# francescoalemanno/KissABC.jl

Hardware: AMD Instinct MI355X
Metric: walker proposal+cost evals/sec at N=65536 walkers, D=8 (higher is better)
Workload: dtype f64

## Files before the change

### include/kabc.h

```cpp
#ifndef KABC_H
#define KABC_H

#ifndef __HIPCC_RTC__
#include <stddef.h>
#include <stdint.h>
#else
#include "kabc_rtc_types.h"
#endif

#ifdef __cplusplus
extern "C" {
#endif

#define KABC_VERSION 321
#define KABC_MAX_DIM 16
#define KABC_MAX_DIM_DYN 256

typedef enum kabc_status {
    KABC_OK = 0,
    KABC_ERR_INVALID_ARG = 1,
    KABC_ERR_RETRY_EXHAUSTED = 2,
    KABC_ERR_INVALID_STATE = 3,
    KABC_ERR_DEVICE = 4,
    KABC_ERR_UNSUPPORTED = 5,
// ... 97 lines not shown
    int64_t keep;
    uint64_t seed;
    int64_t first_row;
} kabc_reject_opts_t;

typedef struct kabc_reject_result {
    double* theta;
    double* cost;
    double* logprior;
    int64_t* index;
    int64_t capacity;
    int64_t n_out;
    int64_t draws;
    int64_t accepted_seen;
    double eps;
    int32_t exhausted;
    int32_t course;
    int64_t launches;
    double kernel_ms;
} kabc_reject_result_t;

void kabc_reject_default_opts(kabc_reject_opts_t* opts);
kabc_status_t kabc_abc_reject(kabc_ctx_t* ctx, const kabc_prior_t* prior, int32_t D, const kabc_cost_t* cost,
                              const kabc_reject_opts_t* opts, kabc_reject_result_t* result);

kabc_status_t kabc_abc_reject_batch(kabc_ctx_t* ctx, const kabc_prior_t* prior, int32_t D,
                                    const kabc_cost_t* costs, int64_t nruns, const uint64_t* seeds,
                                    const double* eps, const kabc_reject_opts_t* opts,
                                    kabc_reject_result_t* results, kabc_status_t* status);
void kabc_reject_batch_stats(int64_t out[4]);

kabc_status_t kabc_math_probe(kabc_ctx_t* ctx, int32_t fn, int64_t n, const double* x,
                              double* out);

kabc_status_t kabc_poison_probe(kabc_ctx_t* ctx, int64_t n, uint8_t* fresh, uint8_t* pooled,
                                uint8_t* recycled, int32_t info[2]);

kabc_status_t kabc_register_cost_plugin(const char* path, int32_t* out_cost_id);
kabc_status_t kabc_compile_cost_plugin(const char* src, const int32_t* dims, int32_t ndims,
                                       int32_t posterior_mask, int32_t* out_cost_id);
kabc_status_t kabc_plugin_precompile(int32_t cost_id, int32_t family, int32_t D, int32_t variant);

kabc_status_t kabc_compile_prior_plugin(const char* src, int32_t discrete, int32_t* out_kind);

kabc_status_t kabc_compile_mvprior_plugin(const char* src, int32_t* out_kind);

#define KABC_FAMILY_AIS 1
#define KABC_FAMILY_SMC 2
#define KABC_FAMILY_ABCDE 4
#define KABC_FAMILY_PFILTER 8
#define KABC_FAMILY_AIS_SMALL 16
kabc_status_t kabc_compile_model(const kabc_model_t* model, int32_t families, int32_t* out_handle);
kabc_status_t kabc_model_release(int32_t handle);
kabc_status_t kabc_prefetch_model(const kabc_model_t* model, int32_t families);
#define KABC_SPECIALIZE_ENV (-1)
#define KABC_SPECIALIZE_OFF 0
#define KABC_SPECIALIZE_BLOCKING 1
#define KABC_SPECIALIZE_BACKGROUND 2
kabc_status_t kabc_set_specialize(int32_t mode);
int32_t kabc_rtc_cache_dir(char* out, int32_t cap);
#define KABC_SPEC_NONE 0
#define KABC_SPEC_PENDING 1
#define KABC_SPEC_ACTIVE 2
#define KABC_SPEC_FAILED 3
kabc_status_t kabc_spec_counters(uint64_t out[4]);
int32_t kabc_rtc_worker_main(const char* jobfile);
// ... 280 lines not shown
```

### kissabc.jl_amd/_cdefs.py

```python
import ctypes as C

KABC_MAX_DIM = 16
KABC_MAX_DIM_DYN = 256
KABC_VERSION = 321
KABC_COMM_ID_BYTES = 128
KABC_MAX_EXCHANGE_CHUNKS = 16
KABC_COMM_MAX_WORLD = 16
COMM_RCCL, COMM_P2P = 1, 2

KABC_OK, KABC_ERR_INVALID_ARG, KABC_ERR_RETRY_EXHAUSTED, KABC_ERR_INVALID_STATE, \
    KABC_ERR_DEVICE, KABC_ERR_UNSUPPORTED, KABC_ERR_NAN_COST, KABC_ERR_CANCELLED = range(8)

PRIOR_UNIFORM, PRIOR_NORMAL, PRIOR_TRUNCNORMAL, PRIOR_BETA, PRIOR_DISCRETE_UNIFORM, \
    PRIOR_NEGBINOMIAL, PRIOR_EXPONENTIAL, PRIOR_GAMMA, PRIOR_LOGNORMAL = range(1, 10)
PRIOR_USER_INIT = 10
PRIOR_MVNORMAL = 11
PRIOR_USER = 100
FAMILY_AIS, FAMILY_SMC, FAMILY_ABCDE, FAMILY_PFILTER, FAMILY_AIS_SMALL = 1, 2, 4, 8, 16

POSTERIOR_KERNELIZED, POSTERIOR_THRESHOLD, POSTERIOR_COMMON = 1, 2, 3
SUMMARY_AUTO, SUMMARY_FULL, SUMMARY_DIAG = 0, 1, 2

COST_GAUSS_DIST, COST_ROSENBROCK, COST_HIER_GAUSS_SIM, COST_NORMAL_MEANSTD_SIM, COST_DIRAC_SQ, \
    COST_ABS_DIFF, COST_NORM_SHELL, COST_NOISY_QUAD_DU, COST_MIXTURE, COST_NOISY_BANANA, \
# ... 92 lines not shown

class RejectOpts(C.Structure):
    _fields_ = [("eps", C.c_double), ("n_accept", C.c_int64), ("max_draws", C.c_int64), ("keep", C.c_int64),
                ("seed", C.c_uint64), ("first_row", C.c_int64)]


class RejectResult(C.Structure):
    _fields_ = [("theta", c_double_p), ("cost", c_double_p), ("logprior", c_double_p),
                ("index", C.POINTER(C.c_int64)), ("capacity", C.c_int64), ("n_out", C.c_int64),
                ("draws", C.c_int64), ("accepted_seen", C.c_int64), ("eps", C.c_double),
                ("exhausted", C.c_int32), ("course", C.c_int32), ("launches", C.c_int64),
                ("kernel_ms", C.c_double)]


ABI_REJECT_OPTS, ABI_REJECT_RESULT = 32, 33

VP = C.c_void_p
PROTOTYPES = {
    "kabc_version": (C.c_int32, []),
    "kabc_abi_sizeof": (C.c_int32, [C.c_int32]),
    "kabc_abi_offsetof": (C.c_int32, [C.c_int32, C.c_int32]),
    "kabc_mvnormal_register": (C.c_int, [c_double_p, c_double_p, C.c_int32, C.POINTER(C.c_int32)]),
    "kabc_last_error": (C.c_char_p, []),
    "kabc_device_count": (C.c_int32, []),
    "kabc_ctx_create": (C.c_int, [C.c_int32, VP, C.POINTER(VP)]),
    "kabc_ctx_destroy": (C.c_int, [VP]),
    "kabc_ctx_synchronize": (C.c_int, [VP]),
    "kabc_ctx_cancel": (C.c_int, [VP]),
    "kabc_ctx_clear_cancel": (C.c_int, [VP]),
    "kabc_ctx_cancel_on_sigint": (C.c_int, [VP, C.c_int32]),
    "kabc_math_probe": (C.c_int, [VP, C.c_int32, C.c_int64, c_double_p, c_double_p]),
    "kabc_poison_probe": (C.c_int, [VP, C.c_int64, C.POINTER(C.c_uint8), C.POINTER(C.c_uint8),
                                    C.POINTER(C.c_uint8), C.POINTER(C.c_int32)]),
    "kabc_host_alloc": (C.c_int, [C.c_size_t, C.POINTER(VP)]),
    "kabc_host_free": (C.c_int, [VP]),
    "kabc_factored_logpdf": (C.c_int, [VP, C.POINTER(Prior), C.c_int32, C.c_int64, c_double_p,
                                       c_double_p]),
    "kabc_factored_push_p": (C.c_int, [VP, C.POINTER(Prior), C.c_int32, C.c_int64, c_double_p,
                                       c_double_p]),
    "kabc_factored_rand": (C.c_int, [VP, C.POINTER(Prior), C.c_int32, C.c_uint64, C.c_uint32,
                                     C.c_int64, C.c_int64, C.c_uint64, c_double_p]),
    "kabc_cost_eval": (C.c_int, [VP, C.POINTER(Cost), C.c_int32, C.c_int64, c_double_p, C.c_int32,
                                 C.c_uint64, C.c_int64, c_double_p]),
    "kabc_prior_predictive": (C.c_int, [VP, C.POINTER(Prior), C.c_int32, C.POINTER(Cost), C.c_int64,
                                        C.c_int32, C.c_uint64, C.c_int64, c_double_p, c_double_p,
                                        c_double_p]),
    "kabc_eval_stats": (None, [c_double_p]),
    "kabc_reject_default_opts": (None, [C.POINTER(RejectOpts)]),
    "kabc_abc_reject": (C.c_int, [VP, C.POINTER(Prior), C.c_int32, C.POINTER(Cost), C.POINTER(RejectOpts),
                                  C.POINTER(RejectResult)]),
    "kabc_abc_reject_batch": (C.c_int, [VP, C.POINTER(Prior), C.c_int32, C.POINTER(Cost), C.c_int64,
                                        C.POINTER(C.c_uint64), c_double_p, C.POINTER(RejectOpts),
                                        C.POINTER(RejectResult), C.POINTER(C.c_int)]),
    "kabc_reject_batch_stats": (None, [C.POINTER(C.c_int64)]),
    "kabc_register_cost_plugin": (C.c_int, [C.c_char_p, C.POINTER(C.c_int32)]),
    "kabc_plugin_precompile": (C.c_int, [C.c_int32, C.c_int32, C.c_int32, C.c_int32]),
    "kabc_compile_cost_plugin": (C.c_int, [C.c_char_p, C.POINTER(C.c_int32), C.c_int32, C.c_int32,
                                         C.POINTER(C.c_int32)]),
    "kabc_compile_prior_plugin": (C.c_int, [C.c_char_p, C.c_int32, C.POINTER(C.c_int32)]),
    "kabc_compile_mvprior_plugin": (C.c_int, [C.c_char_p, C.POINTER(C.c_int32)]),
    "kabc_compile_model": (C.c_int, [C.POINTER(Model), C.c_int32, C.POINTER(C.c_int32)]),
    "kabc_model_release": (C.c_int, [C.c_int32]),
    "kabc_prefetch_model": (C.c_int, [C.POINTER(Model), C.c_int32]),
    "kabc_spec_counters": (C.c_int, [C.POINTER(C.c_uint64)]),
    "kabc_set_specialize": (C.c_int, [C.c_int32]),
    "kabc_rtc_cache_dir": (C.c_int32, [C.c_char_p, C.c_int32]),
# ... 100 lines not shown
```

### kissabc.jl_amd/csrc/ais_inst.hip

```cpp
#define KABC_FMA_C_VGPR
#include "ais_small_kernel.hpp"

#ifndef KABC_INST_COST
#error "compile with -DKABC_INST_COST=<cost id>"
#endif

namespace kabc {

template <int D, int COST, int PC, int PK>
static void launch_half(const AisArgs& a, hipStream_t s, unsigned nchains) {
    const unsigned grid = (unsigned)((a.rows_owned + kBatch - 1) / kBatch);
    if (grid == 0) return;
    hipLaunchKernelGGL((ais_half_kernel<D, COST, PC, PK>), dim3(grid, nchains), dim3(kAisBlock), 0, s, a);
}

template <int D, int COST, int PC, int PK, int K, int NC>
static void launch_half_wide(const AisArgs& a, hipStream_t s, unsigned nchains) {
    const dim3 grid = ais_wide_geom(a, nchains);
    if (grid.x == 0) return;
    hipLaunchKernelGGL((ais_half_wide_kernel<D, COST, PC, PK, K, NC>), grid, dim3(kWideBlock), 0, s, a);
}

#ifndef KABC_INST_DLO
#define KABC_INST_DLO 1
#endif
#ifndef KABC_INST_DHI
#define KABC_INST_DHI KABC_MAX_DIM
#endif
#ifndef KABC_INST_SUFFIX
#define KABC_INST_SUFFIX
#endif
#ifndef KABC_INST_PCSEL
#define KABC_INST_PCSEL 0
#endif
template <int COST, int D, int PCX>
static AisLaunchFn pick() {
    constexpr bool is_normal = (PCX % kPriorClasses) == kPriorNormal;
    constexpr bool pc_ok = KABC_INST_PCSEL == 0 || (KABC_INST_PCSEL == 1) == is_normal;
    if constexpr (pc_ok && D >= KABC_INST_DLO && D <= KABC_INST_DHI && cost_dim_ok_c(COST, D))
        return &launch_half<D, COST, PCX % kPriorClasses, PCX / kPriorClasses + 1>;
    else return nullptr;
}

template <int COST, int D, int PCX>
static AisLaunchFn pick_wide() {
    constexpr bool is_normal = (PCX % kPriorClasses) == kPriorNormal;
    constexpr bool pc_ok = KABC_INST_PCSEL == 0 || (KABC_INST_PCSEL == 1) == is_normal;
    if constexpr (pc_ok && D >= KABC_INST_DLO && D <= KABC_INST_DHI && cost_dim_ok_c(COST, D) &&
                  ais_wide_ok_c(COST, D))
        return &launch_half_wide<D, COST, PCX % kPriorClasses, PCX / kPriorClasses + 1, kWideK, kWideNC>;
    else return nullptr;
}

template <int COST, int PCX, bool WIDE, int... Ds>
static AisLaunchFn row(int D, std::integer_sequence<int, Ds...>) {
    AisLaunchFn f[] = {(WIDE ? pick_wide<COST, Ds + 1, PCX>() : pick<COST, Ds + 1, PCX>())...};
    return (D >= 1 && D <= (int)sizeof...(Ds)) ? f[D - 1] : nullptr;
}

template <int COST, bool WIDE, int... PCXs>
static AisLaunchFn table(int D, int pcx, std::integer_sequence<int, PCXs...>) {
    using Dims = std::make_integer_sequence<int, KABC_MAX_DIM>;
    AisLaunchFn r = nullptr;
    ((pcx == PCXs ? (void)(r = row<COST, PCXs, WIDE>(D, Dims{})) : (void)0), ...);
    return r;
}

template <int COST, int D, int PCX>
static AisSmallLaunchFn pick_small() {
    constexpr int pc = PCX % kPriorClasses;
    constexpr bool is_normal = pc == kPriorNormal;
    constexpr bool pc_ok = KABC_INST_PCSEL == 0 || (KABC_INST_PCSEL == 1) == is_normal;
    if constexpr (pc_ok && pc != kPriorSimple && D >= KABC_INST_DLO &&
                  D <= KABC_INST_DHI && cost_dim_ok_c(COST, D))
        return &launch_ais_small<D, COST, pc, PCX / kPriorClasses + 1>;
    else return nullptr;
}
template <int COST, int PCX, int... Ds>
static AisSmallLaunchFn row_small(int D, std::integer_sequence<int, Ds...>) {
    AisSmallLaunchFn f[] = {pick_small<COST, Ds + 1, PCX>()...};
    return (D >= 1 && D <= (int)sizeof...(Ds)) ? f[D - 1] : nullptr;
}
template <int COST, int... PCXs>
// ... 23 lines not shown
```

### kissabc.jl_amd/csrc/ais_kernels.hpp

```cpp
#pragma once

#include "kabc_device.hpp"
#ifndef __HIPCC_RTC__
#include "launcher.hpp"
#endif

namespace kabc {

struct AisArgs {
    double* x_act;
    const double* x_comp;
    double* lp;
    double* ll;
    double* trace;
    int32_t* dbg;
    DevCounters* counters;
    unsigned long long* slots;
    const double* cost_params;
    const double* cost_data;
    int64_t cost_ndata;
    int64_t row_first;
    int64_t rows_owned;
    int64_t n_comp;
    uint64_t seed;
// ... 23 lines not shown
constexpr int kCounterSlots = 1024;

struct InitArgs {
    double* x_act;
    double* lp;
    double* ll;
    DevCounters* counters;
    const double* cost_params;
    const double* cost_data;
    int64_t cost_ndata;
    int64_t row_first;
    int64_t rows_owned;
    uint64_t seed;
    uint32_t id_base;
    int32_t posterior;
    int32_t cost_id;
    double eps;
    unsigned long long retry_budget;
    PriorSet prior;
    kabc_prior_t raw[KABC_MAX_DIM];
    const uint64_t* seeds;
    unsigned long long* chain_retries;
    int64_t stride_act, stride_own;
    int64_t params_stride, data_stride;
};

constexpr int kInitBlock = 64;

constexpr int kAisBlock = 256;
constexpr int kBatch = 64;
constexpr int kChunk = 3;

struct HalfGeom {
    static constexpr bool kWide = false;
    static constexpr int kBlock = kAisBlock, kBatches = 1, kCh = kChunk, kNC = -1;
};
template <int K, int NC>
struct WideGeom {
    static_assert(K >= 1 && K <= 8 && NC <= K, "the consumer spells out up to 8 sub-steps");
    static constexpr bool kWide = true;
    static constexpr int kBlock = 512, kBatches = 2, kCh = K, kNC = NC;
};
constexpr int kWideBlock = 512, kWideBatches = 2;

template <int D>
struct RecGeom {
    static constexpr int NB = (D + 2) / 2;
    static constexpr int NZ = (D + 2 > 4) ? (D + 2) : 4;
};

template <int Q>
struct SubStepIx {
    static constexpr int value = Q;
};

template <int D, int CH>
struct RecBuf {
    uint32_t mva[CH][kBatch];
    uint32_t bb[CH][kBatch];
    uint32_t cc[CH][kBatch];
    double logu[CH][kBatch];
    double zs[CH][RecGeom<D>::NZ][kBatch];
};
template <int D>
using ChunkRec = RecBuf<D, kChunk>;

enum { kPriorBox = 0, kPriorSimple = 1, kPriorGeneral = 2, kPriorNormal = 3 };
constexpr int kPriorClasses = 4;
constexpr int kNbTabsGeneral = kNbLg1Block;

struct BoxPrior {
    const double* lo;
    const double* hi;
    uint32_t dmask;
    double lp;
};
// ... 366 lines not shown
    const bool consumer = G::kWide ? wave < NBAT : wave == 0;
    const bool tprobe = (KABL & 128) && A.dbg;
    unsigned long long t_begin = 0, t_bar = 0;
    if (tprobe) t_begin = __builtin_amdgcn_s_memtime();
#define KABC_TIMED_BARRIER()                                              \
    do {                                                                  \
        if (tprobe) {                                                     \
            const unsigned long long tb_ = __builtin_amdgcn_s_memtime(); \
            __syncthreads();                                              \
            t_bar += __builtin_amdgcn_s_memtime() - tb_;                  \
        } else {                                                          \
            __syncthreads();                                              \
        }                                                                 \
    } while (0)

    auto comp_row = [&](uint32_t idx) -> const double* {
        return reinterpret_cast<const double*>(reinterpret_cast<const char*>(A.x_comp) +
                                               (size_t)(idx * (uint32_t)(D * sizeof(double))));
    };
    const bool active = consumer && (lane < n_active);
    const int64_t r = r0 + lane;
    const int64_t row = A.row_first + r;
    double x[D];
    double lp = 0.0, ll = 0.0;
    unsigned int n_eval = 0, n_acc = 0;
    int err = 0;
    if (active) {
        load_row<D>(A.x_act + row * D, x);
        lp = A.lp[r];
        ll = A.ll[r];
        if (!ld_valid(PK, lp, ll)) err = 2;
    }

    static_assert(KABC_MATH_TAB_WORDS == 2 * kAisBlock && (G::kBlock == kAisBlock || G::kBlock == 2 * kAisBlock),
                  "two table words per thread, or one");
    const double tab0 = kabc_log_tab[threadIdx.x];
    [[maybe_unused]] double tab1 = 0.0;
    if constexpr (G::kBlock == kAisBlock) tab1 = kabc_log_tab[threadIdx.x + kAisBlock];
    if (threadIdx.x < D * (int)(sizeof(PriorDev) / 8))
        reinterpret_cast<double*>(sprior)[threadIdx.x] =
            reinterpret_cast<const double*>(A.prior)[threadIdx.x];
    if (threadIdx.x < D) {
        sbox_lo[threadIdx.x] = A.prior[threadIdx.x].p[0];
        sbox_hi[threadIdx.x] = A.prior[threadIdx.x].p[1];
    }
    uint32_t dmask = 0, gmask = 0;
    for (int k = 0; k < D; ++k) {
        dmask |= (A.prior[k].discrete ? 1u : 0u) << k;
        gmask |= (gaussbox_is_gauss(A.prior[k].kind) ? 1u : 0u) << k;
    }
    if constexpr (kGaussBox) {
        if (threadIdx.x < D) gaussbox_stage(sgb[threadIdx.x], A.prior[threadIdx.x]);
    }
    const GaussBoxPrior gbox = {sgb, gmask, dmask};
    constexpr bool kBoxRegs = (PC == kPriorBox) && D <= 8;
    double blo[kBoxRegs ? D : 1], bhi[kBoxRegs ? D : 1];
    const BoxPrior box = {kBoxRegs ? blo : sbox_lo, kBoxRegs ? bhi : sbox_hi, dmask, A.box_lp};

    [[maybe_unused]] kabc_u128_t pro01[2] = {};
    if constexpr (!G::kWide) {
        if (wave > 0 && wave - 1 < A.nt && lane < n_active) {
            const uint32_t w = w_base + (uint32_t)lane;
            const uint64_t t = A.t0 + (uint64_t)(wave - 1);
            pro01[0] = kabc_stream_block(A.seed, w, t, 0u, KABC_DOM_AIS_MOVE);
            pro01[1] = kabc_stream_block(A.seed, w, t, 1u, KABC_DOM_AIS_MOVE);
        }
    }
    slogtab[threadIdx.x] = tab0;
    if constexpr (G::kBlock == kAisBlock) slogtab[threadIdx.x + kAisBlock] = tab1;
    if constexpr (G::kWide) {
        uint32_t hw;
        asm volatile("s_getreg_b32 %0, hwreg(HW_REG_HW_ID)" : "=s"(hw));
        if (lane == 0) ssimd[wave] = (hw >> 4) & 3u;
    }
#ifdef KABC_MODEL_SPEC
    [[maybe_unused]] const bool nb_on = kNbTabs > 0;
#else
    [[maybe_unused]] const bool nb_on = kNbTabs > 0 && A.nt >= 8;
#endif
    if constexpr (kNbTabs > 0) {
        static_assert(kNbEntries == kAisBlock, "one table entry per thread (of the first 256)");
        const bool nb_thread = !G::kWide || threadIdx.x < (unsigned)kNbEntries;
        int slot = 0;
        bool has_nb = false;
        for (int k = 0; k < D; ++k) {
            if (A.prior[k].kind == KABC_PRIOR_NEGBINOMIAL) {
                has_nb = true;
                if (nb_on && slot < kNbTabs) {
                    if (nb_thread)
                        snb[slot * kNbEntries + threadIdx.x] =
                            kabc_lgamma_t((double)threadIdx.x + A.prior[k].p[0], kabc_log_tab);
                    ++slot;
                }
            }
        }
        if (has_nb && nb_thread) snb[kNbLg1Block * kNbEntries + threadIdx.x] = kabc_lgamma1_tab[threadIdx.x];
    }
    KABC_TIMED_BARRIER();
    if constexpr (kNbTabs > 0) {
        if (threadIdx.x < D && sprior[threadIdx.x].kind == KABC_PRIOR_NEGBINOMIAL) {
            int slot = 0;
            for (int k = 0; k < (int)threadIdx.x; ++k)
                slot += (sprior[k].kind == KABC_PRIOR_NEGBINOMIAL) ? 1 : 0;
            sprior[threadIdx.x].p[2] = (nb_on && slot < kNbTabs) ? (double)slot : -1.0;
        }
    }
    if constexpr (kBoxRegs) {
#pragma unroll
        for (int k = 0; k < D; ++k) {
            blo[k] = sbox_lo[k];
            bhi[k] = sbox_hi[k];
        }
    }

    uint64_t seed_v = A.seed;
    asm volatile("" : "+v"(seed_v));
    constexpr bool kLate = D > kLateFrom;
    double r0a[D], r0b[D], r1a[kLate ? 1 : D], r1b[kLate ? 1 : D];
    const bool pro_rows = !G::kWide && !(KABL & 5);
    [[maybe_unused]] uint32_t my_tasks = 0;
    if constexpr (G::kWide) {
        constexpr int NT = 2 * CH;
        uint32_t sd = 0;
#pragma unroll
        for (int w = 0; w < NBAT + NPROD; ++w)
            sd |= (uint32_t)__builtin_amdgcn_readfirstlane((int)ssimd[w]) << (4 * w);
        const uint32_t sc0 = sd & 15u, sc1 = (sd >> 4) & 15u;
        uint32_t cot = 0;
        int n0 = 0, n1 = 0;
#pragma unroll
        for (int p = 0; p < NPROD; ++p) {
            const uint32_t sp = (sd >> (4 * (NBAT + p))) & 15u;
            n0 += sp == sc0 ? 1 : 0;
            n1 += sp == sc1 ? 1 : 0;
            cot |= (sp == sc0 || sp == sc1) ? 1u << p : 0u;
        }
        const bool by_place = G::kNC >= 0 && sc0 != sc1 && n0 == 1 && n1 == 1;
        uint32_t cap = 0;
        if (by_place) {
            constexpr int nc = G::kNC >= 0 ? G::kNC : 0;
            constexpr int rest = NT - 2 * nc, others = NPROD - 2;
            int seen = 0;
#pragma unroll
            for (int p = 0; p < NPROD; ++p) {
                int n = nc;
                if (!((cot >> p) & 1u)) {
                    n = rest / others + (seen < rest % others ? 1 : 0);
                    ++seen;
                }
                cap |= (uint32_t)n << (4 * p);
            }
        } else {
#pragma unroll
            for (int p = 0; p < NPROD; ++p) cap |= (uint32_t)(NT / NPROD + (p < NT % NPROD ? 1 : 0)) << (4 * p);
        }
        int p = 0;
        for (int task = 0; task < NT; ++task) {
            while (((cap >> (4 * p)) & 15u) == 0u) p = p + 1 < NPROD ? p + 1 : 0;
            if (p == wave - NBAT) my_tasks |= 1u << task;
            cap -= 1u << (4 * p);
            p = p + 1 < NPROD ? p + 1 : 0;
        }
    }
    auto fill = [&](int buf, int b, int si, int s, int pw, int64_t rb, int nact, uint32_t wb,
                    const kabc_u128_t* pre01, auto mid) __attribute__((always_inline)) {
        produce_substep<D>(A, seed_v, rec[buf][b], si, A.t0 + (uint64_t)s, wb, nact, listB[pw], lane, slogtab,
                           pre01, mid);
        if constexpr (kAuxW > 0)
            prepare_cost_aux<COST, kAuxW>(A, A.t0 + (uint64_t)s, wb, lane, saux[buf][b][si], slogtab, rb, nact);
        if constexpr (kPre > 0)
            produce_cost_normals<kPre>(seed_v, A.t0 + (uint64_t)s, wb, lane, spre[buf][b][si], slogtab);
    };
    [[maybe_unused]] auto fill_tasks = [&](int buf, int sbase) __attribute__((always_inline)) {
#pragma unroll 1
        for (uint32_t m = my_tasks; m != 0u; m &= m - 1u) {
            const int task = __builtin_ctz(m);
            const int si = task >> 1, b = task & 1;
            const int64_t rb = r0_wg + b * kBatch, left = A.rows_owned - rb;
            if (sbase + si < A.nt && left > 0)
                fill(buf, b, si, sbase + si, wave - NBAT, rb, left >= kBatch ? kBatch : (int)left,
                     A.id_base + (uint32_t)(A.row_first + rb), nullptr, NoMid());
        }
    };
    if constexpr (G::kWide) {
        if (!consumer && !(KABL & 4)) fill_tasks(0, 0);
    } else if (wave > 0) {
        const int si = wave - 1;
        if (si < A.nt && !(KABL & 4)) {
            fill(0, 0, si, si, si, r0, n_active, w_base, pro01, [] { __syncthreads(); });
        } else {
            __syncthreads();
        }
    } else {
        __syncthreads();
#ifndef KABC_NO_XCHUNK_PREFETCH
// ... 193 lines not shown
        if (active) {
            store_row<D>(A.x_act + row * D, x);
            A.lp[r] = lp;
            A.ll[r] = ll;
            if (A.trace) {
                double xp[D];
#pragma unroll
                for (int k = 0; k < D; ++k)
                    xp[k] = (sprior[k].discrete && PK != KABC_POSTERIOR_COMMON)
                                ? kabc_rint(x[k]) : x[k];
                store_row<D>(A.trace + r * D, xp);
            }
        }
        const unsigned long long se = wave_total_u32(n_eval);
        const unsigned long long sa = wave_total_u32(n_acc);
        if (lane == 0 && (!G::kWide || n_active > 0)) {
            unsigned long long* sl =
                A.slots + (size_t)((blockIdx.x * NBAT + bmine + blockIdx.y * gridDim.x * NBAT) & (kCounterSlots - 1)) * 8;
            atomicAdd(&sl[0], (unsigned long long)n_active * (unsigned long long)A.nt);
            atomicAdd(&sl[1], se);
            atomicAdd(&sl[2], sa);
        }
        if (err) atomicMax(&A.counters->error, err);
    }
#undef KABC_TIMED_BARRIER
}

template <int D, int COST, int PC, int PK>
__global__ void __launch_bounds__(kAisBlock) __attribute__((amdgpu_waves_per_eu(2, 2)))
ais_half_kernel(const AisArgs A0) {
    ais_half_body<D, COST, PC, PK, HalfGeom>(A0);
}

template <int D, int COST, int PC, int PK, int K, int NC>
__global__ void __launch_bounds__(kWideBlock) __attribute__((amdgpu_waves_per_eu(2, 2)))
ais_half_wide_kernel(const AisArgs A0) {
    ais_half_body<D, COST, PC, PK, WideGeom<K, NC>>(A0);
}

template <int D>
__global__ void __launch_bounds__(kInitBlock) ais_init_kernel(const InitArgs A) {
    const int64_t r = (int64_t)blockIdx.x * kInitBlock + threadIdx.x;
    if (r >= A.rows_owned) return;
    const int64_t row = A.row_first + r;
    const uint32_t w = A.id_base + (uint32_t)row;
    const int64_t chain = (int64_t)blockIdx.y;
    const uint64_t seed = A.seeds ? A.seeds[chain] : A.seed;
    unsigned long long* retries = A.seeds ? A.chain_retries + chain : &A.counters->retries;
    double* x_act = A.x_act + (A.seeds ? chain * A.stride_act : 0);
    double* lp_out = A.lp + (A.seeds ? chain * A.stride_own : 0);
    double* ll_out = A.ll + (A.seeds ? chain * A.stride_own : 0);
    const double* cparams = A.cost_params + (A.seeds ? chain * A.params_stride : 0);
    const double* cdata = A.cost_data + (A.seeds ? chain * A.data_stride : 0);
    double x[D], xp[D];
    double lp = 0.0, ll = 0.0;
    uint64_t attempt = 0;
    while (true) {
#ifdef KABC_USER_SAMPLE_INIT
        if (A.raw[0].kind == KABC_PRIOR_USER_INIT) {
            kabc_cost_rng_t irng = {seed, attempt, w, KABC_DOM_AIS_INIT, 0u};
            kabc_user_sample_init(x, D, cparams, cdata, A.cost_ndata, &irng);
        } else
#endif
        {
            for (int k = 0; k < D; ++k) {
                kabc_slotwin_t win = {seed, attempt, w, KABC_DOM_AIS_INIT,
                                      (uint32_t)k * KABC_SLOTS_PER_DIM};
                x[k] = kabc_sample_prior(&A.raw[k], &win);
            }
        }
// ... 8 lines not shown
                const double c = kabc_cost_eval(A.cost_id, xp, D, cparams, cdata, A.cost_ndata, &rng);
                const double q = kabc_div_rc(c, A.eps, 1.0 / A.eps);
                ll = -0.5 * (q * q);
            }
        } else {
            ll = -lp;
            if (kabc_isfinite(lp))
                ll = kabc_cost_eval(A.cost_id, xp, D, cparams, cdata, A.cost_ndata, &rng);
        }
        if (ld_valid(A.posterior, lp, ll)) break;
        const unsigned long long used = atomicAdd(retries, 1ull) + 1ull;
        if (used > A.retry_budget) {
            A.counters->init_failed = 1;
            break;
        }
        ++attempt;
    }
    store_row<D>(x_act + row * D, x);
    lp_out[r] = lp;
    ll_out[r] = ll;
}

#ifndef __HIPCC_RTC__
using AisLaunchFn = void (*)(const AisArgs&, hipStream_t, unsigned nchains);
using AisLaunch = Launcher<AisArgs, unsigned>;
using AisInitLaunch = Launcher<InitArgs, unsigned>;
inline dim3 ais_half_geom(const AisArgs& a, unsigned nchains) {
    return dim3((unsigned)((a.rows_owned + kBatch - 1) / kBatch), nchains);
}
inline dim3 ais_init_geom(const InitArgs& a, unsigned nchains) {
    return dim3((unsigned)((a.rows_owned + kInitBlock - 1) / kInitBlock), nchains);
}
AisLaunch find_ais_kernel(int cost_id, int D, int pcx);
constexpr int kWideK = 4, kWideNC = 1;
constexpr int kWideMaxDim = 8;
constexpr bool ais_wide_ok_c(int cost, int D) {
    const int nz = (D + 2 > 4) ? (D + 2) : 4;
    if (D > kWideMaxDim) return false;
    return cost < KABC_COST_USER && cost_aux_c(cost) == 0 && ais_pre_blocks(cost, D) == 0 &&
           4 * kWideK * kBatch * (20 + 8 * nz) + (12 << 10) <= (160 << 10);
}
inline dim3 ais_wide_geom(const AisArgs& a, unsigned nchains) {
    return dim3((unsigned)((a.rows_owned + kWideBatches * kBatch - 1) / (kWideBatches * kBatch)), nchains);
}
AisLaunch find_ais_wide_kernel(int cost_id, int D, int pcx);
constexpr int kAisVariants = 3 * kPriorClasses;
struct ModelUnit;
bool launch_ais_init(int D, const InitArgs& a, hipStream_t s, unsigned nchains, ModelUnit* unit);

#endif

}
```

### kissabc.jl_amd/csrc/capi_ais.hip

```cpp
#include <chrono>
#include <condition_variable>
#include <cstdio>
#include <cstdlib>
#include <mutex>
#include <thread>
#include <type_traits>
#include <vector>

#include "ais_aux_kernels.hpp"
#include "ais_dyn_kernels.hpp"
#include "ais_dyn_small_kernel.hpp"
#include "ais_small_kernel.hpp"
#include "ais_summary_kernel.hpp"
#include "host_common.hpp"
#include "plugin_registry.hpp"

namespace kabc {

#define KABC_DECL_COST(id)                                                \
    AisLaunchFn find_ais_kernel_cost_##id(int D, int pc);                 \
    AisLaunchFn find_ais_kernel_cost_##id##_nrm(int D, int pc);           \
    AisLaunchFn find_ais_kernel_cost_##id##_hi(int D, int pc);            \
    AisLaunchFn find_ais_wide_kernel_cost_##id(int D, int pc);            \
    AisLaunchFn find_ais_wide_kernel_cost_##id##_nrm(int D, int pc);      \
// ... 995 lines not shown
        e = hipEventCreate(&x.x0[k]);
        if (e == hipSuccess) e = hipEventCreate(&x.x1[k]);
    }
    if (e != hipSuccess) xt_release(x, xk);
    return e;
}

static void timing_release(kabc_ais_t* h) {
    for (hipEvent_t e : h->ev) (void)hipEventDestroy(e);
    h->ev.clear();
    for (const kabc_ais::XT& x : h->xt) xt_release(x, h->xk);
    h->xt.clear();
}

static void ais_poll_spec(kabc_ais_t* h) {
    const auto now = std::chrono::steady_clock::now();
    if (now < h->spec_next_poll) return;
    h->spec_next_poll = now + std::chrono::milliseconds(2);
    int st = KABC_SPEC_NONE;
    const PluginKernel k = unit_kernel(h->unit, h->small_ok ? kPfAisSmall : kPfAis, h->D, h->spec_variant, &st);
    if (st == KABC_SPEC_ACTIVE && k.mod) {
        if (h->small_ok) h->small = AisSmallLaunch(k.mod, &ais_small_geom, (unsigned)kAisSmallBlock);
        else {
            h->launch = AisLaunch(k.mod, &ais_half_geom, (unsigned)kAisBlock);
            h->launch_wide = nullptr;
        }
        h->spec_state = KABC_SPEC_ACTIVE;
        h->spec_switch_at = h->launches;
    } else if (st == KABC_SPEC_FAILED) {
        h->spec_state = KABC_SPEC_FAILED;
    }
}

constexpr int32_t kAisWideFrom = 32;
static bool ais_can_wide(const kabc_ais_t* h, int64_t rows) {
    return h->launch_wide && h->nchains == 1 && h->world == 1 && !h->comm && rows >= kWideBatches * kBatch;
}
static int64_t ais_wide_min_rows() {
    static const int64_t v = [] {
        int dev = 0, cus = 0;
        if (hipGetDevice(&dev) != hipSuccess ||
            hipDeviceGetAttribute(&cus, hipDeviceAttributeMultiprocessorCount, dev) != hipSuccess || cus < 1)
            cus = 256;
        return (int64_t)kWideBatches * kBatch * cus;
    }();
    return v;
}
static bool ais_use_wide(const kabc_ais_t* h, int64_t rows, int32_t nt) {
    if (!ais_can_wide(h, rows)) return false;
    const char* e = std::getenv("KABC_AIS_WIDE");
    if (e && e[0]) return e[0] != '0';
    return nt >= kAisWideFrom && rows >= ais_wide_min_rows();
}

static kabc_status_t launch_half_seg(kabc_ais_t* h, int32_t half, const kabc_ais::Seg& sg,
                                     int32_t ntransitions, double* dev_trace_rows) {
    if (sg.count == 0) return KABC_OK;
    hipStream_t s = h->ctx->stream;
    if (h->spec_state == KABC_SPEC_PENDING && !h->small_ok) ais_poll_spec(h);
    if (!h->launch && !h->dyn)
        if (kabc_status_t st = ais_resolve_half(h)) return st;
    if (h->dyn && h->nchains > 1) {
        set_error("a handle of %d chains beyond %d parameters advances with kabc_ais_advance (the one-workgroup "
                  "driver); kabc_ais_half_generation drives one chain per handle there", h->nchains, KABC_MAX_DIM);
        return KABC_ERR_UNSUPPORTED;
    }
    if (!h->dyn && !ais_can_wide(h, sg.count)) {
// ... 44 lines not shown
                if (v) fprintf(stderr, "[kabc] KABC_ABLATE=%d ignored: the timing probes are compiled "
                                       "only into libkabc_hip_probes.so (make PROBES=1, KABC_PROBES=1)\n", v);
#endif
                return v;
            }();
            a.ablate = ab;
        }
        const int W = aux_prepass_words(h->cost_id);
        int32_t blk = ntransitions;
        if (W) {
            const size_t per_step = sizeof(double) * (size_t)W * (size_t)sg.count * (size_t)h->nchains;
            const size_t cap = env_bytes("KABC_AUX_KIB", 1 << 10, (size_t)256 << 20);
            const size_t fit = cap / per_step;
            blk = (int32_t)(fit < 1 ? 1 : (fit > (size_t)ntransitions ? (size_t)ntransitions : fit));
            if (kabc_status_t st = grow(h, &h->d_aux, &h->aux_cap, per_step * (size_t)blk)) return st;
        }
        for (int32_t s0 = 0; s0 < ntransitions; s0 += blk) {
            const int32_t nb = ntransitions - s0 < blk ? ntransitions - s0 : blk;
            a.t0 = h->t + (uint64_t)s0;
            a.nt = nb;
            a.dbg_s0 = s0;
            a.trace = (dev_trace_rows && s0 + nb == ntransitions) ? dev_trace_rows + sg.off * h->D : nullptr;
            if (W) {
                a.aux = h->d_aux;
                a.stride_aux = enqueue_aux(h, half, sg.first, sg.count, a.t0, nb, h->d_aux);
            }
            (ais_use_wide(h, sg.count, nb) ? h->launch_wide : h->launch)(a, s, (unsigned)h->nchains);
        }
    }
    if (t_on && ++h->open_count >= h->timing_stride)
        if (kabc_status_t st = timing_close_pair(h)) return st;
    KABC_HIP_CHECK(hipGetLastError());
    return KABC_OK;
}

kabc_status_t kabc_ais_half_generation(kabc_ais_t* h, int32_t half, int32_t ntransitions,
                                       void* dev_trace_rows) {
    if (check_handle(h)) return KABC_ERR_INVALID_ARG;
    if (!h->initialised) {
        set_error("kabc_ais_init / kabc_ais_set_state has not been called");
        return KABC_ERR_INVALID_STATE;
    }
    if ((half != 0 && half != 1) || ntransitions < 1) {
        set_error("half must be 0/1 and ntransitions >= 1");
        return KABC_ERR_INVALID_ARG;
    }
    if (kabc_status_t st = counter_room(h, 1, ntransitions, "kabc_ais_half_generation")) return st;
    for (const kabc_ais::Seg& sg : h->seg[half])
        if (kabc_status_t st = launch_half_seg(h, half, sg, ntransitions, (double*)dev_trace_rows))
            return st;
    return KABC_OK;
}

kabc_status_t kabc_ais_end_generation(kabc_ais_t* h, int32_t ntransitions) {
    if (check_handle(h)) return KABC_ERR_INVALID_ARG;
    if (kabc_status_t st = counter_room(h, 1, ntransitions, "kabc_ais_end_generation")) return st;
    h->t += (uint64_t)ntransitions;
    return KABC_OK;
}

}

static int64_t ais_small_units_per_gen(const kabc_ais_t* h, int32_t ntransitions) {
    if (h->dsmall) {
        const int64_t teams = h->dplan.block / h->dplan.T;
        const int64_t rounds = (h->rows[0] + teams - 1) / teams + (h->rows[1] + teams - 1) / teams;
// ... 976 lines not shown
```

Measured before the change: 30.90 billion.

## Run wide AIS kernel with twelve waves and larger chunks for small D

The wide AIS kernel now takes the wave count as a template parameter and uses 12 waves (three per SIMD) for low dimensions, with chunk 6 and two co-located tasks. The task-dealing logic moves into a shared host/device function so it handles more waves, and the wide path kicks in from 24 transitions instead of 32. The aim is more latency hiding and producer parallelism per workgroup. In exchange the kernel holds fewer registers per wave (one set of partner rows), does late row loads, and uses more LDS.

```diff
diff --git a/include/kabc.h b/include/kabc.h
--- a/include/kabc.h
+++ b/include/kabc.h
@@ -153,6 +153,10 @@
 
 kabc_status_t kabc_math_probe(kabc_ctx_t* ctx, int32_t fn, int64_t n, const double* x,
                               double* out);
+
+kabc_status_t kabc_ais_wide_deal(const int32_t* simd, int32_t waves, int32_t chunk, int32_t nc,
+                                 uint32_t* masks);
+void kabc_ais_wide_shipped(int32_t geom[3]);
 
 kabc_status_t kabc_poison_probe(kabc_ctx_t* ctx, int64_t n, uint8_t* fresh, uint8_t* pooled,
                                 uint8_t* recycled, int32_t info[2]);
diff --git a/kissabc.jl_amd/_cdefs.py b/kissabc.jl_amd/_cdefs.py
--- a/kissabc.jl_amd/_cdefs.py
+++ b/kissabc.jl_amd/_cdefs.py
@@ -148,6 +148,9 @@
     "kabc_math_probe": (C.c_int, [VP, C.c_int32, C.c_int64, c_double_p, c_double_p]),
     "kabc_poison_probe": (C.c_int, [VP, C.c_int64, C.POINTER(C.c_uint8), C.POINTER(C.c_uint8),
                                     C.POINTER(C.c_uint8), C.POINTER(C.c_int32)]),
+    "kabc_ais_wide_deal": (C.c_int, [C.POINTER(C.c_int32), C.c_int32, C.c_int32, C.c_int32,
+                                     C.POINTER(C.c_uint32)]),
+    "kabc_ais_wide_shipped": (None, [C.POINTER(C.c_int32)]),
     "kabc_host_alloc": (C.c_int, [C.c_size_t, C.POINTER(VP)]),
     "kabc_host_free": (C.c_int, [VP]),
     "kabc_factored_logpdf": (C.c_int, [VP, C.POINTER(Prior), C.c_int32, C.c_int64, c_double_p,
diff --git a/kissabc.jl_amd/csrc/ais_inst.hip b/kissabc.jl_amd/csrc/ais_inst.hip
--- a/kissabc.jl_amd/csrc/ais_inst.hip
+++ b/kissabc.jl_amd/csrc/ais_inst.hip
@@ -14,11 +14,11 @@
     hipLaunchKernelGGL((ais_half_kernel<D, COST, PC, PK>), dim3(grid, nchains), dim3(kAisBlock), 0, s, a);
 }
 
-template <int D, int COST, int PC, int PK, int K, int NC>
+template <int D, int COST, int PC, int PK, int K, int NC, int W>
 static void launch_half_wide(const AisArgs& a, hipStream_t s, unsigned nchains) {
     const dim3 grid = ais_wide_geom(a, nchains);
     if (grid.x == 0) return;
-    hipLaunchKernelGGL((ais_half_wide_kernel<D, COST, PC, PK, K, NC>), grid, dim3(kWideBlock), 0, s, a);
+    hipLaunchKernelGGL((ais_half_wide_kernel<D, COST, PC, PK, K, NC, W>), grid, dim3(W * 64), 0, s, a);
 }
 
 #ifndef KABC_INST_DLO
@@ -48,7 +48,9 @@
     constexpr bool pc_ok = KABC_INST_PCSEL == 0 || (KABC_INST_PCSEL == 1) == is_normal;
     if constexpr (pc_ok && D >= KABC_INST_DLO && D <= KABC_INST_DHI && cost_dim_ok_c(COST, D) &&
                   ais_wide_ok_c(COST, D))
-        return &launch_half_wide<D, COST, PCX % kPriorClasses, PCX / kPriorClasses + 1, kWideK, kWideNC>;
+        return &launch_half_wide<D, COST, PCX % kPriorClasses, PCX / kPriorClasses + 1,
+                                 ais_wide_chunk_c(D, PCX % kPriorClasses), ais_wide_nc_c(D, PCX % kPriorClasses),
+                                 ais_wide_waves_c(D, PCX % kPriorClasses)>;
     else return nullptr;
 }
 
diff --git a/kissabc.jl_amd/csrc/ais_kernels.hpp b/kissabc.jl_amd/csrc/ais_kernels.hpp
--- a/kissabc.jl_amd/csrc/ais_kernels.hpp
+++ b/kissabc.jl_amd/csrc/ais_kernels.hpp
@@ -79,16 +79,71 @@
 constexpr int kChunk = 3;
 
 struct HalfGeom {
-    static constexpr bool kWide = false;
+    static constexpr bool kWide = false, kOneRowSet = false;
     static constexpr int kBlock = kAisBlock, kBatches = 1, kCh = kChunk, kNC = -1;
 };
-template <int K, int NC>
+constexpr int kWideBatches = 2, kWideMaxWaves = 12;
+template <int K, int NC, int W = 8, bool ONE = (W > 8)>
 struct WideGeom {
     static_assert(K >= 1 && K <= 8 && NC <= K, "the consumer spells out up to 8 sub-steps");
-    static constexpr bool kWide = true;
-    static constexpr int kBlock = 512, kBatches = 2, kCh = K, kNC = NC;
+    static_assert(W == 8 || W == 12, "two or three waves on each of the four SIMDs");
+    static_assert(W == 8 || ONE, "three waves per SIMD have registers for one set of partner rows");
+    static constexpr bool kWide = true, kOneRowSet = ONE;
+    static constexpr int kWaves = W, kBlock = W * 64, kBatches = kWideBatches, kCh = K, kNC = NC;
 };
-constexpr int kWideBlock = 512, kWideBatches = 2;
+
+#ifdef __HIP_DEVICE_COMPILE__
+#define KABC_DEAL_UNROLL _Pragma("unroll")
+#else
+#define KABC_DEAL_UNROLL
+#endif
+__host__ __device__ __forceinline__ uint32_t wide_deal_mask(uint64_t sd, int W, int K, int nc, int me) {
+    const int NPROD = W - kWideBatches, NT = 2 * K, beside = W / 4 - 1;
+    const uint32_t sc0 = (uint32_t)sd & 15u, sc1 = (uint32_t)(sd >> 4) & 15u;
+    uint32_t cot = 0;
+    int n0 = 0, n1 = 0;
+    KABC_DEAL_UNROLL
+    for (int p = 0; p < NPROD; ++p) {
+        const uint32_t sp = (uint32_t)(sd >> (4 * (kWideBatches + p))) & 15u;
+        n0 += sp == sc0 ? 1 : 0;
+        n1 += sp == sc1 ? 1 : 0;
+        cot |= (sp == sc0 || sp == sc1) ? 1u << p : 0u;
+    }
+    const bool by_place = nc >= 0 && sc0 != sc1 && n0 == beside && n1 == beside;
+    uint64_t cap = 0;
+    if (by_place) {
+        const int rest = NT - 2 * nc, others = NPROD - 2 * beside;
+        int seen = 0, seen0 = 0, seen1 = 0;
+    KABC_DEAL_UNROLL
+        for (int p = 0; p < NPROD; ++p) {
+            int n;
+            if ((cot >> p) & 1u) {
+                const bool on0 = ((uint32_t)(sd >> (4 * (kWideBatches + p))) & 15u) == sc0;
+                const int k = on0 ? seen0 : seen1;
+                n = nc / beside + (k < nc % beside ? 1 : 0);
+                seen0 += on0 ? 1 : 0;
+                seen1 += on0 ? 0 : 1;
+            } else {
+                n = rest / others + (seen < rest % others ? 1 : 0);
+                ++seen;
+            }
+            cap |= (uint64_t)n << (4 * p);
+        }
+    } else {
+    KABC_DEAL_UNROLL
+        for (int p = 0; p < NPROD; ++p) cap |= (uint64_t)(NT / NPROD + (p < NT % NPROD ? 1 : 0)) << (4 * p);
+    }
+    uint32_t mine = 0;
+    int p = 0;
+    for (int task = 0; task < NT; ++task) {
+        while (((cap >> (4 * p)) & 15u) == 0u) p = p + 1 < NPROD ? p + 1 : 0;
+        if (p == me) mine |= 1u << task;
+        cap -= (uint64_t)1 << (4 * p);
+        p = p + 1 < NPROD ? p + 1 : 0;
+    }
+    return mine;
+}
+#undef KABC_DEAL_UNROLL
 
 template <int D>
 struct RecGeom {
@@ -521,9 +576,10 @@
         if (!ld_valid(PK, lp, ll)) err = 2;
     }
 
-    static_assert(KABC_MATH_TAB_WORDS == 2 * kAisBlock && (G::kBlock == kAisBlock || G::kBlock == 2 * kAisBlock),
-                  "two table words per thread, or one");
-    const double tab0 = kabc_log_tab[threadIdx.x];
+    static_assert(KABC_MATH_TAB_WORDS == 2 * kAisBlock && (G::kBlock == kAisBlock || G::kBlock >= 2 * kAisBlock),
+                  "two table words per thread, or one for each of the first 512");
+    const bool tab_thread = G::kBlock <= KABC_MATH_TAB_WORDS || threadIdx.x < (unsigned)KABC_MATH_TAB_WORDS;
+    const double tab0 = tab_thread ? kabc_log_tab[threadIdx.x] : 0.0;
     [[maybe_unused]] double tab1 = 0.0;
     if constexpr (G::kBlock == kAisBlock) tab1 = kabc_log_tab[threadIdx.x + kAisBlock];
     if (threadIdx.x < D * (int)(sizeof(PriorDev) / 8))
@@ -555,7 +611,7 @@
             pro01[1] = kabc_stream_block(A.seed, w, t, 1u, KABC_DOM_AIS_MOVE);
         }
     }
-    slogtab[threadIdx.x] = tab0;
+    if (tab_thread) slogtab[threadIdx.x] = tab0;
     if constexpr (G::kBlock == kAisBlock) slogtab[threadIdx.x + kAisBlock] = tab1;
     if constexpr (G::kWide) {
         uint32_t hw;
@@ -604,52 +660,17 @@
 
     uint64_t seed_v = A.seed;
     asm volatile("" : "+v"(seed_v));
-    constexpr bool kLate = D > kLateFrom;
+    constexpr bool kLate = D > kLateFrom || G::kOneRowSet;
     double r0a[D], r0b[D], r1a[kLate ? 1 : D], r1b[kLate ? 1 : D];
     const bool pro_rows = !G::kWide && !(KABL & 5);
     [[maybe_unused]] uint32_t my_tasks = 0;
     if constexpr (G::kWide) {
-        constexpr int NT = 2 * CH;
-        uint32_t sd = 0;
+        static_assert(4 * (NBAT + NPROD) <= 64, "the SIMD ids of a workgroup's waves, four bits apiece");
+        uint64_t sd = 0;
 #pragma unroll
         for (int w = 0; w < NBAT + NPROD; ++w)
-            sd |= (uint32_t)__builtin_amdgcn_readfirstlane((int)ssimd[w]) << (4 * w);
-        const uint32_t sc0 = sd & 15u, sc1 = (sd >> 4) & 15u;
-        uint32_t cot = 0;
-        int n0 = 0, n1 = 0;
-#pragma unroll
-        for (int p = 0; p < NPROD; ++p) {
-            const uint32_t sp = (sd >> (4 * (NBAT + p))) & 15u;
-            n0 += sp == sc0 ? 1 : 0;
-            n1 += sp == sc1 ? 1 : 0;
-            cot |= (sp == sc0 || sp == sc1) ? 1u << p : 0u;
-        }
-        const bool by_place = G::kNC >= 0 && sc0 != sc1 && n0 == 1 && n1 == 1;
-        uint32_t cap = 0;
-        if (by_place) {
-            constexpr int nc = G::kNC >= 0 ? G::kNC : 0;
-            constexpr int rest = NT - 2 * nc, others = NPROD - 2;
-            int seen = 0;
-#pragma unroll
-            for (int p = 0; p < NPROD; ++p) {
-                int n = nc;
-                if (!((cot >> p) & 1u)) {
-                    n = rest / others + (seen < rest % others ? 1 : 0);
-                    ++seen;
-                }
-                cap |= (uint32_t)n << (4 * p);
-            }
-        } else {
-#pragma unroll
-            for (int p = 0; p < NPROD; ++p) cap |= (uint32_t)(NT / NPROD + (p < NT % NPROD ? 1 : 0)) << (4 * p);
-        }
-        int p = 0;
-        for (int task = 0; task < NT; ++task) {
-            while (((cap >> (4 * p)) & 15u) == 0u) p = p + 1 < NPROD ? p + 1 : 0;
-            if (p == wave - NBAT) my_tasks |= 1u << task;
-            cap -= 1u << (4 * p);
-            p = p + 1 < NPROD ? p + 1 : 0;
-        }
+            sd |= (uint64_t)(uint32_t)__builtin_amdgcn_readfirstlane((int)ssimd[w]) << (4 * w);
+        my_tasks = wide_deal_mask(sd, NBAT + NPROD, CH, G::kNC, wave - NBAT);
     }
     auto fill = [&](int buf, int b, int si, int s, int pw, int64_t rb, int nact, uint32_t wb,
                     const kabc_u128_t* pre01, auto mid) __attribute__((always_inline)) {
@@ -909,10 +930,10 @@
     ais_half_body<D, COST, PC, PK, HalfGeom>(A0);
 }
 
-template <int D, int COST, int PC, int PK, int K, int NC>
-__global__ void __launch_bounds__(kWideBlock) __attribute__((amdgpu_waves_per_eu(2, 2)))
+template <int D, int COST, int PC, int PK, int K, int NC, int W = 8, bool ONE = (W > 8)>
+__global__ void __launch_bounds__(W * 64) __attribute__((amdgpu_waves_per_eu(W / 4, W / 4)))
 ais_half_wide_kernel(const AisArgs A0) {
-    ais_half_body<D, COST, PC, PK, WideGeom<K, NC>>(A0);
+    ais_half_body<D, COST, PC, PK, WideGeom<K, NC, W, ONE>>(A0);
 }
 
 template <int D>
@@ -987,13 +1008,26 @@
     return dim3((unsigned)((a.rows_owned + kInitBlock - 1) / kInitBlock), nchains);
 }
 AisLaunch find_ais_kernel(int cost_id, int D, int pcx);
-constexpr int kWideK = 4, kWideNC = 1;
+constexpr int kWideK = 6, kWideNC = 2, kWideW = 12;
+constexpr int kWideBlock = kWideW * 64;
+constexpr int kWideW8 = 8, kWideK8 = 4, kWideNC8 = 1;
+constexpr int ais_wide_waves_c(int D, int pc) {
+    const int dmax = pc == kPriorBox ? 8 : pc == kPriorNormal ? 6 : pc == kPriorSimple ? 4 : 2;
+    return D <= dmax ? kWideW : kWideW8;
+}
+constexpr int ais_wide_chunk_c(int D, int pc) { return ais_wide_waves_c(D, pc) == kWideW ? kWideK : kWideK8; }
+constexpr int ais_wide_nc_c(int D, int pc) { return ais_wide_waves_c(D, pc) == kWideW ? kWideNC : kWideNC8; }
 constexpr int kWideMaxDim = 8;
+constexpr int ais_wide_lds_c(int D, int pc) {
+    const int nz = (D + 2 > 4) ? (D + 2) : 4;
+    return 4 * ais_wide_chunk_c(D, pc) * kBatch * (20 + 8 * nz) + (ais_wide_waves_c(D, pc) - kWideBatches) * kBatch +
+           ((pc == kPriorGeneral ? 12 : 6) << 10);
+}
 constexpr bool ais_wide_ok_c(int cost, int D) {
-    const int nz = (D + 2 > 4) ? (D + 2) : 4;
     if (D > kWideMaxDim) return false;
     return cost < KABC_COST_USER && cost_aux_c(cost) == 0 && ais_pre_blocks(cost, D) == 0 &&
-           4 * kWideK * kBatch * (20 + 8 * nz) + (12 << 10) <= (160 << 10);
+           ais_wide_lds_c(D, kPriorBox) <= (160 << 10) && ais_wide_lds_c(D, kPriorSimple) <= (160 << 10) &&
+           ais_wide_lds_c(D, kPriorGeneral) <= (160 << 10) && ais_wide_lds_c(D, kPriorNormal) <= (160 << 10);
 }
 inline dim3 ais_wide_geom(const AisArgs& a, unsigned nchains) {
     return dim3((unsigned)((a.rows_owned + kWideBatches * kBatch - 1) / (kWideBatches * kBatch)), nchains);
diff --git a/kissabc.jl_amd/csrc/capi_ais.hip b/kissabc.jl_amd/csrc/capi_ais.hip
--- a/kissabc.jl_amd/csrc/capi_ais.hip
+++ b/kissabc.jl_amd/csrc/capi_ais.hip
@@ -1051,7 +1051,7 @@
     }
 }
 
-constexpr int32_t kAisWideFrom = 32;
+constexpr int32_t kAisWideFrom = 24;
 static bool ais_can_wide(const kabc_ais_t* h, int64_t rows) {
     return h->launch_wide && h->nchains == 1 && h->world == 1 && !h->comm && rows >= kWideBatches * kBatch;
 }
@@ -1162,6 +1162,29 @@
         if (kabc_status_t st = timing_close_pair(h)) return st;
     KABC_HIP_CHECK(hipGetLastError());
     return KABC_OK;
+}
+
+kabc_status_t kabc_ais_wide_deal(const int32_t* simd, int32_t waves, int32_t chunk, int32_t nc,
+                                 uint32_t* masks) {
+    if (!simd || !masks || (waves != 8 && waves != 12) || chunk < 1 || chunk > 8 || nc > chunk) {
+        set_error("kabc_ais_wide_deal: bad argument (waves 8 or 12, chunk 1..8, nc <= chunk)");
+        return KABC_ERR_INVALID_ARG;
+    }
+    uint64_t sd = 0;
+    for (int w = 0; w < waves; ++w) {
+        if (simd[w] < 0 || simd[w] > 15) {
+            set_error("kabc_ais_wide_deal: SIMD id %d of wave %d is not in 0..15", (int)simd[w], w);
+            return KABC_ERR_INVALID_ARG;
+        }
+        sd |= (uint64_t)simd[w] << (4 * w);
+    }
+    for (int p = 0; p < waves - kWideBatches; ++p) masks[p] = wide_deal_mask(sd, waves, chunk, nc, p);
+    return KABC_OK;
+}
+void kabc_ais_wide_shipped(int32_t geom[3]) {
+    geom[0] = kWideW;
+    geom[1] = kWideK;
+    geom[2] = kWideNC;
 }
 
 kabc_status_t kabc_ais_half_generation(kabc_ais_t* h, int32_t half, int32_t ntransitions,
```

After: 33.04 billion, median of 6. 6.9% higher.
